# AugmentariumLab/VolumeRenderer

Measured on AMD Instinct MI355X. Metric: Mvoxels/s kd-tree compress+decode, higher is better.
Workload: dtype u8; 1 GPU; 2048x2048x1920 uint8 volume per GPU as 960 bricks of 256x256x128, rm_volume, tolerance 1, maxEpochs 2, VolumeKdtree build + levelCut

## Files before the change

### include/vrhip.h

```cpp
#ifndef VRHIP_H
#define VRHIP_H

#include <stdint.h>

#ifdef __cplusplus
extern "C" {
#endif

typedef int32_t vr_status;
enum {
    VR_OK = 0,
    VR_ERR_INVALID = -1,
    VR_ERR_NO_DEVICE = -2,
    VR_ERR_OOM = -3,
    VR_ERR_IO = -4,
    VR_ERR_STATE = -5,
    VR_ERR_FORMAT = -6,
    VR_ERR_UNSUPPORTED = -7
};

enum {
    VR_VARIANT_RECOVER = 0,
    VR_VARIANT_GUARDED = 1,
    VR_VARIANT_MIDRANGE = 2
// ... 267 lines not shown
vr_status vr_stream_create(void **stream);
vr_status vr_stream_destroy(void *stream);
vr_status vr_stream_synchronize(void *stream);
vr_status vr_stream_wait_event(void *stream, void *event);
vr_status vr_event_create(void **event);
vr_status vr_event_destroy(void *event);
vr_status vr_event_record(void *event, void *stream);
vr_status vr_event_synchronize(void *event);
vr_status vr_event_elapsed_ms(void *start_event, void *end_event, float *ms);
vr_status vr_malloc_host(void **host, int64_t bytes);
vr_status vr_free_host(void *host);
vr_status vr_upload_async(void *dst_dev, const void *src_host, int64_t bytes, void *stream);
vr_status vr_download_async(void *dst_host, const void *src_dev, int64_t bytes, void *stream);

vr_status vr_brickset_last_timings(vr_brickset *bs, float phases_ms[5]);

vr_status vr_brickset_set_concurrency(vr_brickset *bs, int32_t level_loop_streams);

vr_status vr_brickset_set_compaction(vr_brickset *bs, int32_t on_build);

vr_status vr_brickset_set_switch(vr_brickset *bs, const char *name, int32_t value);
vr_status vr_debug_set(const char *name, int32_t value);

#ifdef __cplusplus
}
#endif
#endif
```

### volumerenderer_amd/_lib.py

```python
import ctypes as C
import os

HERE = os.path.dirname(os.path.abspath(__file__))
LIB_PATH = os.path.join(HERE, "libvrhip.so")

VR_OK = 0
STATUS = {0: "VR_OK", -1: "VR_ERR_INVALID", -2: "VR_ERR_NO_DEVICE", -3: "VR_ERR_OOM", -4: "VR_ERR_IO",
          -5: "VR_ERR_STATE", -6: "VR_ERR_FORMAT", -7: "VR_ERR_UNSUPPORTED"}
VARIANT_RECOVER, VARIANT_GUARDED, VARIANT_MIDRANGE = 0, 1, 2
RENDER_COMPOSITE, RENDER_ISOSURFACE, RENDER_PARTIAL, RENDER_SHADED, RENDER_PROJECTION = 0, 1, 2, 3, 4
PROJECT_MAX, PROJECT_MIN, PROJECT_MEAN = 0, 1, 2
SLICE_NEAREST, SLICE_LINEAR = 0, 1


class VrError(RuntimeError):
    def __init__(self, status, what=""):
        self.status = status
        super().__init__("%s: %s (%d)" % (what, STATUS.get(status, "?"), status))


class TreeInfo(C.Structure):
    _fields_ = [("X", C.c_int64), ("Y", C.c_int64), ("Z", C.c_int64),
                ("orig_tree_depth", C.c_int32), ("max_tree_depth", C.c_int32),
                ("num_active_nodes", C.c_int64), ("tree_bytes", C.c_int64),
                ("tolerance", C.c_int32), ("max_epochs", C.c_int32), ("variant", C.c_int32),
                ("num_reverts", C.c_int32), ("max_error_before", C.c_int32), ("max_error_after", C.c_int32),
                ("mean_l1_after", C.c_double), ("zero_run_rewrites", C.c_int32), ("est_exact_segments", C.c_int32)]


class Camera(C.Structure):
    _fields_ = [("pos", C.c_float * 3), ("front", C.c_float * 3), ("up", C.c_float * 3),
                ("fov_deg", C.c_float), ("z_near", C.c_float), ("z_far", C.c_float)]


class RenderParams(C.Structure):
# ... 118 lines not shown
    "vr_compositor_create_from_comm": (_I32, [C.POINTER(_P), _P, _I32, _I32, _I32, _I32]),
    "vr_compositor_create_with_transport": (_I32, [C.POINTER(_P), _P, _P, _I32, _I32, _I32, _I32]),
    "vr_compositor_composite": (_I32, [_P, _P, _I32, C.POINTER(Camera), C.POINTER(RenderParams), _P, _P]),
    "vr_compositor_composite_tf": (_I32, [_P, _P, _I32, C.POINTER(Camera), C.POINTER(RenderParams),
                                          C.POINTER(TransferFunctionDesc), _P, _P]),
    "vr_compositor_composite_proj": (_I32, [_P, _P, C.POINTER(Projection), _P, _P]),
    "vr_compositor_destroy": (_I32, [_P]),
    "vr_stream_create": (_I32, [C.POINTER(_P)]),
    "vr_stream_destroy": (_I32, [_P]),
    "vr_stream_synchronize": (_I32, [_P]),
    "vr_stream_wait_event": (_I32, [_P, _P]),
    "vr_event_create": (_I32, [C.POINTER(_P)]),
    "vr_event_destroy": (_I32, [_P]),
    "vr_event_record": (_I32, [_P, _P]),
    "vr_event_synchronize": (_I32, [_P]),
    "vr_event_elapsed_ms": (_I32, [_P, _P, C.POINTER(C.c_float)]),
    "vr_malloc_host": (_I32, [C.POINTER(_P), _I64]),
    "vr_free_host": (_I32, [_P]),
    "vr_upload_async": (_I32, [_P, _P, _I64, _P]),
    "vr_download_async": (_I32, [_P, _P, _I64, _P]),
    "vr_brickset_last_timings": (_I32, [_P, C.POINTER(C.c_float)]),
    "vr_brickset_set_concurrency": (_I32, [_P, C.c_int32]),
    "vr_brickset_set_switch": (_I32, [_P, C.c_char_p, C.c_int32]),
    "vr_brickset_set_compaction": (_I32, [_P, C.c_int32]),
    "vr_debug_set": (_I32, [C.c_char_p, C.c_int32]),
}

_lib = None


def lib():
    global _lib
    if _lib is None:
        if not os.path.exists(LIB_PATH):
            raise ImportError("libvrhip.so is missing: run `python -c 'import __graft_entry__ as g; g.build()'` "
                              "(hipcc --offload-arch=gfx950).  There is no CPU fallback.")
        import torch
        L = C.CDLL(LIB_PATH)
        for name, (res, args) in SIGNATURES.items():
            fn = getattr(L, name)
            fn.restype = res
            fn.argtypes = args
        _lib = L
    return _lib


# ... 4 lines not shown
```

### volumerenderer_amd/codec.py

```python
import ctypes as C
import os

import numpy as np
import torch

from . import _lib
from ._lib import VrError, check


def _stream_ptr(stream=None):
    s = stream if stream is not None else torch.cuda.current_stream()
    return C.c_void_p(s.cuda_stream)


def _as_dev_u8(x):
    if isinstance(x, np.ndarray):
        x = torch.from_numpy(np.ascontiguousarray(x, dtype=np.uint8))
    if not isinstance(x, torch.Tensor) or x.dtype != torch.uint8:
        raise TypeError("expected a uint8 numpy array or torch tensor")
    if not x.is_cuda:
        x = x.cuda()
    return x.contiguous()


# ... 11 lines not shown
        self.dims = tuple(int(v) for v in dims)
        self.voxels_per_brick = self.dims[0] * self.dims[1] * self.dims[2]
        self._keep = None

    def __del__(self):
        try:
            if self._h:
                self._L.vr_brickset_destroy(self._h)
                self._h = None
        except Exception:
            pass

    def set_error_tolerance(self, tol):
        check(self._L.vr_brickset_set_error_tolerance(self._h, int(tol)), "setErrorTolerance")

    def set_max_epochs(self, e):
        check(self._L.vr_brickset_set_max_epochs(self._h, int(e)), "setMaxEpochs")

    def set_compaction(self, on_build=True):
        check(self._L.vr_brickset_set_compaction(self._h, 1 if on_build else 0), "vr_brickset_set_compaction")

    def set_switch(self, name, value=1):
        check(self._L.vr_brickset_set_switch(self._h, name.encode(), int(value)), "vr_brickset_set_switch(%s)" % name)

    def build(self, voxels, stream=None):
        v = _as_dev_u8(voxels)
        if v.numel() != self.num_bricks * self.voxels_per_brick:
            raise ValueError("voxel buffer has %d bytes, expected %d" % (v.numel(), self.num_bricks * self.voxels_per_brick))
        self._keep = v
        check(self._L.vr_brickset_build(self._h, C.c_void_p(v.data_ptr()), _stream_ptr(stream)), "vr_brickset_build")
        return self

    def info(self, brick=0):
        ti = _lib.TreeInfo()
        check(self._L.vr_brickset_info(self._h, int(brick), C.byref(ti)), "vr_brickset_info")
        return {k: getattr(ti, k) for k, _ in ti._fields_}

    def tree(self, brick=0):
        n = self.info(brick)["tree_bytes"]
        out = np.empty(n, np.uint8)
        check(self._L.vr_brickset_get_tree(self._h, int(brick), out.ctypes.data, n), "vr_brickset_get_tree")
        return out

    def distance_map(self, brick=0):
        n = self.info(brick)["max_tree_depth"] + 1
        out = np.empty(n, np.uint8)
# ... 254 lines not shown
```

### volumerenderer_amd/csrc/brickset.h

```cpp
#pragma once
#include "kd_common.h"
#include "../../include/vrhip.h"
#include <algorithm>
#include <string>
#include <vector>

namespace vr {

struct Stream2 {
    uint8_t *temp = nullptr;
    uint8_t *codes = nullptr;
    uint8_t *recon[3] = {nullptr, nullptr, nullptr};
    Ctrl *ctrl = nullptr;
    uint8_t *tree = nullptr;
    uint8_t *treeCompact = nullptr;
};

#define EST_R0_BUDGET 8
struct Switches {
    bool decodeWalk = false;
    bool decodeFineV1 = false;
    bool decodeQuad = false;
    bool noSkipBlocks = false;
    bool noUniformBlocks = false;
    bool estExactBounds = false;
    int estBudget = EST_R0_BUDGET;
    bool noUniformDecode = false;
};

#define VR_LOD_SLOTS 4
struct LodSlot {
    int32_t *dev = nullptr;
    int32_t *host = nullptr;
    uint8_t *idxValCut = nullptr;
    uint32_t *decTables = nullptr;
    uint8_t *rankVals = nullptr;
    int64_t *obDev = nullptr;
    int64_t *obHost = nullptr;
    vr_pool_entry *tabHost = nullptr;
    int64_t tabCap = 0;
    hipEvent_t done = nullptr;
    bool pending = false;
};

struct BrickSet {
    int32_t B = 0;
    Switches sw;
    Geom g{};
    TilePlan tile{};
// ... 110 lines not shown
```

### volumerenderer_amd/csrc/capi.hip

```cpp
#include "../../include/vrhip.h"
#include "brickset.h"
#include "raymarch.h"
#include <math.h>
#include <stdio.h>
#include <stdlib.h>
#include <string.h>
#include <algorithm>
#include <array>
#include <atomic>
#include <map>
#include <mutex>
#include <new>

using namespace vr;

struct vr_brickset { BrickSet s; };

#define HIPCHK(x) do { hipError_t e_ = (x); if (e_ != hipSuccess) return e_ == hipErrorOutOfMemory ? VR_ERR_OOM : VR_ERR_NO_DEVICE; } while (0)

static bool device_ok()
{
    int n = 0;
    hipError_t e = hipGetDeviceCount(&n);
    if ((e != hipSuccess || n <= 0) && getenv("VRHIP_DEBUG"))
// ... 80 lines not shown
    hipFree(s.treeCompact);
    hipFree(s.temp); hipFree(s.codes);
    for (int i = 0; i < 3; ++i) hipFree(s.recon[i]);
    hipFree(s.ctrl); hipFree(s.tree);
    s = Stream2();
}

static vr_status alloc_stream2(BrickSet &b, Stream2 &s)
{
    const size_t B = (size_t)b.B;
    HIPCHK(hipMalloc(&s.ctrl, B * sizeof(Ctrl)));
    HIPCHK(hipMemset(s.ctrl, 0, B * sizeof(Ctrl)));
    HIPCHK(hipMalloc(&s.tree, B * (size_t)b.treeCap));
    return VR_OK;
}

static void free_encoder_buffers(BrickSet &b)
{
    auto drop = [](auto *&p) { if (p) hipFree(p); p = nullptr; };
    Stream2 *ss[2] = {&b.mid, &b.rng};
    for (Stream2 *s : ss) {
        drop(s->temp); drop(s->codes);
        for (int i = 0; i < 3; ++i) drop(s->recon[i]);
    }
    for (int i = 0; i < 2; ++i) { drop(b.mmMin[i]); drop(b.mmMax[i]); }
    drop(b.blockErr); drop(b.estSumm); drop(b.blockErrR); drop(b.estSummR); drop(b.blockL1); drop(b.blockFlag); drop(b.blockFlagR); drop(b.blockAlive); drop(b.blockVal); drop(b.blockSpine); drop(b.blockSpineR);
    drop(b.chainLut); drop(b.blockTot); drop(b.blockOff); drop(b.blockOff64); drop(b.idxBase);
    b.encoderReady = false;
}

static vr_status alloc_encoder_buffers(BrickSet &b)
{
    const size_t B = (size_t)b.B;
    b.leafless = leafless_build(b);
    b.reconStride = b.leafless ? b.leafStride / 2 : b.leafStride;
    b.codeStride = b.leafless ? b.leafStride / 4 + 16 : ((b.heapStride + 15) / 16) * 4;
    HIPCHK(hipMalloc(&b.mid.temp, B * (size_t)b.heapStride));
    HIPCHK(hipMalloc(&b.mid.codes, B * (size_t)b.codeStride));
    for (int i = 0; i < 3; ++i) HIPCHK(hipMalloc(&b.mid.recon[i], B * (size_t)b.reconStride));
    if (b.variant == VR_VARIANT_MIDRANGE) {
        if (!b.rng.ctrl) HIPCHK(hipMalloc(&b.rng.ctrl, B * sizeof(Ctrl)));
        if (!b.rng.tree) HIPCHK(hipMalloc(&b.rng.tree, B * (size_t)b.treeCap));
        HIPCHK(hipMalloc(&b.rng.temp, B * (size_t)b.heapStride));
        HIPCHK(hipMalloc(&b.rng.codes, B * (size_t)b.codeStride));
        for (int i = 0; i < 3; ++i) HIPCHK(hipMalloc(&b.rng.recon[i], B * (size_t)b.reconStride));
    }
// ... 64 lines not shown
{
    if (!out || !dims || num_bricks <= 0) return VR_ERR_INVALID;
    if (tolerance < 0 || max_epochs < 0 || variant < 0 || variant > 2) return VR_ERR_INVALID;
    for (int k = 0; k < 3; ++k) if (dims[k] <= 0) return VR_ERR_INVALID;
    if (max_epochs > VR_MAX_EPOCHS) return VR_ERR_UNSUPPORTED;
    bool general = !pow2(dims[0]) || !pow2(dims[1]) || !pow2(dims[2]) || dims[0] > 1024 || dims[1] > 1024 || dims[2] > 1024;
    if (dims[0] > (1ll << 20) || dims[1] > (1ll << 20) || dims[2] > (1ll << 20) || dims[0] * dims[1] * dims[2] >= (1ll << 32))
        return VR_ERR_UNSUPPORTED;
    if (!device_ok()) return VR_ERR_NO_DEVICE;
    vr_brickset *h = new (std::nothrow) vr_brickset();
    if (!h) return VR_ERR_OOM;
    BrickSet &b = h->s;
    b.B = num_bricks;
    {
        Switches &w = b.sw;
        w.decodeWalk = getenv("VRHIP_DECODE_WALK") != nullptr;
        w.decodeFineV1 = getenv("VRHIP_DECODE_FINE_V1") != nullptr;
        w.decodeQuad = getenv("VRHIP_DECODE_QUAD") != nullptr;
        w.noSkipBlocks = getenv("VRHIP_NO_SKIP_BLOCKS") != nullptr;
        w.noUniformBlocks = getenv("VRHIP_NO_UNIFORM_BLOCKS") != nullptr;
        w.noUniformDecode = getenv("VRHIP_NO_UNIFORM_DECODE") != nullptr;
        w.estExactBounds = getenv("VRHIP_EST_EXACT_BOUNDS") != nullptr;
        if (const char *eb = getenv("VRHIP_EST_BUDGET")) { const int v = atoi(eb); if (v >= 0) w.estBudget = v; }
    }
    make_geom(b.g, dims);
    b.D = b.g.D;
    if (b.D > 31) { delete h; return VR_ERR_UNSUPPORTED; }
    b.idx64 = b.D > 28 || (getenv("VRHIP_FORCE_IDX64") && b.D >= 12);
    if (b.idx64) general = true;
    if (b.idx64 && num_bricks != 1 && b.D > 28) { delete h; return VR_ERR_UNSUPPORTED; }
    b.generalGeom = general;
    b.maxDepth = b.D + VR_CHAIN_LEVELS;
    b.tolerance = tolerance; b.maxEpochs = max_epochs; b.variant = variant;
    b.K = b.D < 6 ? b.D : 6;
    b.Ds = b.D - b.K;
    b.heapStride = (int64_t)1 << (b.D + 1);
    b.leafStride = (int64_t)1 << b.D;
    b.codeStride = ((b.heapStride + 15) / 16) * 4;
    b.reconStride = b.leafStride;
    const int64_t numMax = b.heapStride - 1 + VR_CHAIN_LEVELS * b.leafStride;
    b.treeCap = ((numMax + 15) / 16 + 2) * 4 + 256;
    if (b.D >= 12) {
        const int64_t gappedBytes = ((int64_t)1 << (b.D - 12)) * 2320 * 4 + 256;
        if (gappedBytes > b.treeCap) b.treeCap = gappedBytes;
    }
    b.nIdx = (int64_t)1 << b.Ds;
// ... 16 lines not shown
        if (e == hipSuccess && !general) e = upload(b.spread, make_spread(b.g));
        for (int i = 0; i < 8 && e == hipSuccess; ++i) e = hipEventCreate(&b.ev[i]);
        if (e != hipSuccess) rc = e == hipErrorOutOfMemory ? VR_ERR_OOM : VR_ERR_NO_DEVICE;
    }
    if (rc != VR_OK) { vr_brickset_destroy(h); return rc; }
    b.hostCtrl.resize(b.B);
    b.openTreeBytes.assign(b.B, -1);
    *out = h;
    return VR_OK;
}

vr_status vr_brickset_set_switch(vr_brickset *h, const char *name, int32_t value)
{
    if (!h || !name) return VR_ERR_INVALID;
    Switches &w = h->s.sw;
    const bool on = value != 0;
    if (!strcmp(name, "decode_walk")) w.decodeWalk = on;
    else if (!strcmp(name, "decode_fine_v1")) w.decodeFineV1 = on;
    else if (!strcmp(name, "decode_quad")) w.decodeQuad = on;
    else if (!strcmp(name, "no_skip_blocks")) w.noSkipBlocks = on;
    else if (!strcmp(name, "no_uniform_blocks")) w.noUniformBlocks = on;
    else if (!strcmp(name, "no_uniform_decode")) w.noUniformDecode = on;
    else if (!strcmp(name, "est_exact_bounds")) w.estExactBounds = on;
    else return VR_ERR_INVALID;
    return VR_OK;
}

vr_status vr_brickset_set_compaction(vr_brickset *h, int32_t on_build)
{
    if (!h) return VR_ERR_INVALID;
    h->s.compactOnBuild = on_build != 0;
    return VR_OK;
}

vr_status vr_debug_set(const char *name, int32_t value)
{
    if (!name) return VR_ERR_INVALID;
    if (!strcmp(name, "skip_grid_v1")) { vr::g_skipGridV1.store(value ? 1 : 0); return VR_OK; }
    if (!strcmp(name, "reslice_tile_w")) {
        if (value != 8 && value != 16 && value != 64) return VR_ERR_INVALID;
        vr::g_resliceTileLog2.store(value == 8 ? 3 : (value == 16 ? 4 : 6));
        return VR_OK;
    }
    if (!strcmp(name, "hist_plain")) { vr::g_histPlain.store(value ? 1 : 0); return VR_OK; }
    return VR_ERR_INVALID;
}

// ... 1018 lines not shown
```

### volumerenderer_amd/csrc/kd_encode.hip

```cpp
#include "brickset.h"
#include <math.h>
#include <stdio.h>
#include <stdlib.h>
#include <string.h>

namespace vr {

#define FILL_NODES_PER_BLOCK 1024
#define EMIT_RANKS_PER_BLOCK 256

template <bool FROM_VOXELS>
__global__ void __launch_bounds__(256)
k_pyramid(Geom g, int dLeaf, int L, const uint8_t *__restrict__ vox, const uint8_t *__restrict__ inMin,
          const uint8_t *__restrict__ inMax, int64_t inStride, uint8_t *__restrict__ temp, int64_t heapStride,
          uint8_t *__restrict__ tempRange, uint8_t *__restrict__ outMin, uint8_t *__restrict__ outMax,
          int64_t outStride, const uint32_t *__restrict__ srcIdx)
{
    __shared__ uint8_t smn[2][1024], smx[2][1024];
    const int brick = blockIdx.y;
    const uint32_t n = 1u << L;
    const uint32_t base = blockIdx.x << L;
    uint8_t *T = temp + (int64_t)brick * heapStride;
    uint8_t *TR = tempRange ? tempRange + (int64_t)brick * heapStride : nullptr;
    for (uint32_t i = threadIdx.x; i < n; i += blockDim.x) {
// ... 259 lines not shown
    if (threadIdx.x) return;
    c.constBrick = 0; c.constVal = 0; c.zeroRun = 0;
    if (rootMin) {
        const int mn = rootMin[(int64_t)blockIdx.x * mmStride], mx = rootMax[(int64_t)blockIdx.x * mmStride];
        c.constBrick = mn == mx ? 1 : 0;
        c.constVal = mn;
    }
    c.currentDistance = c.currentError = c.currentDF = c.currentStepSize = 0.0;
    c.previousDistance = c.previousError = c.previousDF = c.previousStepSize = 0.0;
    c.errMinus = c.errPlus = 0;
    c.statL1 = 0;
    c.numActive = 0;
    c.epoch = 0; c.active = 0; c.fillThisEpoch = 0;
    c.cur = 0; c.prev = 1; c.pendingEqual = 0;
    c.par = 0; c.ra = 1; c.rb = 2;
    c.altValid = 0; c.altSel = 0; c.altDist = 0;
    c.numReverts = 0; c.maxErrBefore = 0; c.maxErrAfter = 0;
    c.estS = 0; c.estC = 0; c.estTbase = 0; c.estFallbacks = 0; c.estSeg = 0; c.estDone = 0; c.emitOverflow = 0;
    for (int i = 0; i < VR_MAX_DEPTH + 8; ++i) c.distanceMap[i] = 0;
}

#define EST_SEG 1024
#define EST_CAND 8
#define EST_ROUNDS 5
#define EST_HEAD 4096

#define est_at(ci, seg) (((int64_t)(ci) * summStride + (int64_t)(seg)) * 4)

__device__ __forceinline__ uint32_t wave_incl_scan_u32(uint32_t v, int lane)
{
    (void)lane;
    return wave_incl_scan_add_dpp(v);
}

__device__ __forceinline__ uint32_t lane_u32(uint32_t v, int l) { return (uint32_t)__builtin_amdgcn_readlane((int)v, l); }
__device__ __forceinline__ unsigned long long lane_u64(unsigned long long v, int l)
{
    return (unsigned long long)lane_u32((uint32_t)v, l) | ((unsigned long long)lane_u32((uint32_t)(v >> 32), l) << 32);
}

#define EST_STAGE_NODES 4096
__device__ inline void est_exact_chain(const uint8_t *__restrict__ T, const uint8_t *__restrict__ P, int d, uint32_t lo,
                                       uint32_t hi, unsigned long long &S, uint32_t &C, int lane, const SkipBlocks &sk, int brick,
                                       uint8_t *stage = nullptr)
{
    const uint32_t len = hi - lo;
    const bool staged = stage && d > 0 && len >= 64u && len <= (uint32_t)EST_STAGE_NODES && (len & 63u) == 0u && (lo & 31u) == 0u;
// ... 88 lines not shown
            c.estDone = 0;
            c.estTbase = est_window_base((long long)(S / (2ull * C + 1ull)), 4);
        }
    }
}

__device__ __forceinline__ uint32_t seg_incl_scan_add_dpp(uint32_t v)
{
    v = row_incl_scan_add_dpp(v);
    return v + dpp_u32<0x142, 0xa>(0, v);
}
__device__ __forceinline__ int seg_max_i32_dpp(int v)
{
    v = row_max_i32_dpp(v);
    return max(v, (int)dpp_u32<0x142, 0xa>(0x80000000u, (uint32_t)v));
}
__device__ __forceinline__ int seg_min_i32_dpp(int v)
{
    v = row_min_i32_dpp(v);
    return min(v, (int)dpp_u32<0x142, 0xa>(0x7FFFFFFFu, (uint32_t)v));
}

template <bool QUADS>
__global__ void __launch_bounds__(256)
k_est_summ(int d, int nc, Ctrl *ctrls, const uint8_t *__restrict__ temp, int64_t heapStride, ReconBufs rb,
           int64_t leafStride, uint32_t *__restrict__ summ, int64_t summStride, SkipBlocks sk)
{
    constexpr int L = 32, SPW = 64 / L, NP = EST_SEG / 2 / L, TW = NP / 2, PW = NP / 4;
    const int brick = blockIdx.y, lane = threadIdx.x & 63, row = lane / L, rl = lane % L;
    const Ctrl &c = ctrls[brick];
    const uint32_t n = 1u << d;
    const int cConst = c.constBrick, cDone = c.estDone, cSeg = c.estSeg, cPar = c.par, cTbase = c.estTbase;
    if (cConst || cDone) return;
    const uint8_t *Tl = temp + (int64_t)brick * heapStride + ((int64_t)1 << d) + rl * (4 * TW);
    const uint8_t *Pl = (cPar == 0 ? rb.b[0] : (cPar == 1 ? rb.b[1] : rb.b[2])) + (int64_t)brick * leafStride + rl * (4 * PW);
    const uint32_t nseg = n / EST_SEG, step = gridDim.x * (4u * SPW);
    const uint32_t g0 = (uint32_t)cSeg + (blockIdx.x * 4u + (threadIdx.x >> 6)) * SPW;
    uint4 tN[TW / 4], pN[PW / 4];
    auto fetch = [&](uint32_t g) {
        const uint32_t s = g + (uint32_t)row;
        const bool live = s < nseg && !skip_block(sk, brick, d, s * EST_SEG);
#pragma unroll
        for (int j = 0; j < TW / 4; ++j) tN[j] = make_uint4(0, 0, 0, 0);
#pragma unroll
        for (int j = 0; j < PW / 4; ++j) pN[j] = make_uint4(0, 0, 0, 0);
        if (live) {
#pragma unroll
            for (int j = 0; j < TW / 4; ++j) tN[j] = ld16(Tl + (size_t)s * EST_SEG + 16 * j);
#pragma unroll
            for (int j = 0; j < PW / 4; ++j) pN[j] = ld16(Pl + (size_t)s * (EST_SEG / 2) + 16 * j);
        }
    };
    fetch(g0);
    const int Tbase = cTbase;
    uint32_t *out = summ + (int64_t)brick * summStride * (4 * EST_CAND);
    for (uint32_t g = g0; g < nseg; g += step) {
    uint32_t tw[TW], pw[PW];
#pragma unroll
    for (int j = 0; j < TW / 4; ++j) { tw[4 * j] = tN[j].x; tw[4 * j + 1] = tN[j].y; tw[4 * j + 2] = tN[j].z; tw[4 * j + 3] = tN[j].w; }
#pragma unroll
// ... 113 lines not shown
                amax = __builtin_elementwise_max(amax, low);
                bmin = __builtin_elementwise_min(bmin, pk_mad(cc, two2, low));
            }
        }
        const int low1 = low.x, low2 = low.y, cc1 = cc.x, cc2 = cc.y;
        lowT = low1 + low2; ccT = cc1 + cc2;
        a = max((int)amax.x, max((int)amax.y, 0) + low1);
        b = min((int)bmin.x, min((int)bmin.y, 0) + low1 + 2 * cc1);
        }
        const uint32_t sT = (uint32_t)(2 * Th * ccT - lowT);
        const uint32_t packed = sT | ((uint32_t)ccT << 20);
        const uint32_t incl = seg_incl_scan_add_dpp(packed), excl = incl - packed;
        const int s0 = (int)(excl & 0xFFFFFu), c0 = (int)(excl >> 20);
        a += 2 * Th * c0 - s0;
        b += 2 * (Th + 1) * c0 - s0;
        a = seg_max_i32_dpp(a);
        b = seg_min_i32_dpp(b);
        if (segLive && rl == L - 1)
            *(uint4 *)(out + est_at(ci, seg)) = make_uint4(incl & 0xFFFFFu, incl >> 20, (uint32_t)a, (uint32_t)b);
    }
    }
}

__global__ void __launch_bounds__(64)
k_est_walk(int d, int maxEpochs, int nc, int ncNext, int lastRound, int budget, Ctrl *ctrls, const uint8_t *__restrict__ temp, int64_t heapStride, ReconBufs rb,
           int64_t leafStride, const uint32_t *__restrict__ summ, int64_t summStride, SkipBlocks sk)
{
    const int brick = blockIdx.x, lane = threadIdx.x;
    Ctrl &c = ctrls[brick];
    const uint8_t *T = temp + (int64_t)brick * heapStride + ((int64_t)1 << d);
    const uint8_t *P = rb.b[c.par] + (int64_t)brick * leafStride;
    const uint32_t n = 1u << d, nseg = n / EST_SEG;
    const uint32_t *sm = summ + (int64_t)brick * summStride * (4 * EST_CAND);
    if (c.constBrick || c.estDone) return;
    __shared__ __attribute__((aligned(16))) uint8_t stage[EST_STAGE_NODES + EST_STAGE_NODES / 2];
    unsigned long long S = c.estS;
    uint32_t C = c.estC;
    const int Tbase = c.estTbase;
    long long Tc = (long long)(S / (2ull * C + 1ull));
    uint32_t seg = (uint32_t)c.estSeg;
    int fallbacks = 0;
    uint32_t preSeg = 0xFFFFFFFFu;
    long long preCi = -1;
    uint4 pre[4];
#pragma unroll
    for (int j = 0; j < 4; ++j) pre[j] = make_uint4(0, 0, 0x80000000u, 0x7FFFFFFFu);
    const auto fetch = [&](long long ci_, uint32_t seg_, uint4 (&r)[4]) {
        const uint32_t k0 = seg_ + 4u * (uint32_t)lane;
#pragma unroll
        for (int j = 0; j < 4; ++j) {
            r[j] = make_uint4(0, 0, 0x80000000u, 0x7FFFFFFFu);
            if (k0 + (uint32_t)j < nseg) r[j] = *(const uint4 *)(sm + est_at((int)ci_, k0 + (uint32_t)j));
        }
    };
    while (seg < nseg) {
        const long long ci = Tc - Tbase;
        if (ci < 0 || ci >= nc || (budget >= 0 && !lastRound && fallbacks > budget)) {
            if (!lastRound) {
                if (lane == 0) {
                    c.estS = S; c.estC = C; c.estSeg = (int)seg;
                    c.estTbase = est_window_base(Tc, ncNext);
                    c.estFallbacks += fallbacks;
                }
                return;
            }
            est_exact_chain(T, P, d, seg * EST_SEG, n, S, C, lane, sk, brick);
            fallbacks += (int)(nseg - seg);
            break;
        }
        uint4 r[4];
        if (preSeg == seg && preCi == ci) {
#pragma unroll
            for (int j = 0; j < 4; ++j) r[j] = pre[j];
        } else fetch(ci, seg, r);
        preSeg = seg + 256u; preCi = ci;
        fetch(ci, preSeg, pre);
        const uint32_t k0 = seg + 4u * (uint32_t)lane;
        const uint32_t ssL = r[0].x + r[1].x + r[2].x + r[3].x, scL = r[0].y + r[1].y + r[2].y + r[3].y;
        const uint32_t si = wave_incl_scan_u32(ssL, lane), sci = wave_incl_scan_u32(scL, lane);
        uint32_t eS = si - ssL, eC = sci - scL;
        int failJ = 4;
        uint32_t fS = 0, fC = 0;
#pragma unroll
        for (int j = 0; j < 4; ++j) {
            const long long S0 = (long long)S + (long long)eS;
// ... 1789 lines not shown
    }
    const int64_t s = (int64_t)blockIdx.x * 256 + threadIdx.x;
    if (s < nIdx) {
        idxOff[(int64_t)brick * nIdx + s] = VR_IDX_DEAD;
        idxVal[(int64_t)brick * nIdx + s] = (uint8_t)v;
    }
}

__global__ void k_const_finish_range(int D, Ctrl *ctrlsR, uint8_t *treeR, int64_t treeCap, const unsigned long long *brickOff = nullptr,
                                     int64_t compactCap = 0)
{
    Ctrl &c = ctrlsR[blockIdx.x];
    if (threadIdx.x || !c.constBrick) return;
    if (brickOff && brickOff[gridDim.x] > (unsigned long long)compactCap) return;
    const int v = c.constVal;
    for (int d = 0; d <= D; ++d) c.distanceMap[d] = 0;
    c.numActive = v ? 3 : 1;
    *(uint32_t *)(treeR + (brickOff ? (int64_t)brickOff[blockIdx.x] : (int64_t)blockIdx.x * treeCap)) = v ? 0x3Cu : 0x03u;
    c.numReverts = 0; c.maxErrBefore = 0; c.maxErrAfter = 0; c.statL1 = 0; c.emitOverflow = 0;
}

static inline unsigned cdiv(int64_t a, int64_t b) { return (unsigned)((a + b - 1) / b); }

static void compress_stream(BrickSet *bs, Stream2 &s0, hipStream_t st, const uint8_t *rootMin, const uint8_t *rootMax,
                            int64_t mmStride, SkipBlocks sk, unsigned long long *blockErr, void *estSumm0,
                            int b0 = 0, int nb = -1)
{
    const int D = bs->D, B = nb < 0 ? bs->B : nb;
    struct { Ctrl *ctrl; uint8_t *temp, *codes; uint8_t *recon[3]; } s;
    s.ctrl = s0.ctrl + b0; s.temp = s0.temp + (int64_t)b0 * bs->heapStride; s.codes = s0.codes + (int64_t)b0 * bs->codeStride;
    for (int i = 0; i < 3; ++i) s.recon[i] = s0.recon[i] + (int64_t)b0 * bs->reconStride;
    blockErr += (int64_t)b0 * bs->nErrBlk;
    const int64_t errPlane = (int64_t)bs->B * bs->nErrBlk;
    void *estSumm = (uint32_t *)estSumm0 + (int64_t)b0 * bs->estSummStride * (4 * EST_CAND);
    if (sk.flag) sk.flag += (int64_t)b0 * sk.nBlk;
    if (rootMin) { rootMin += (int64_t)b0 * mmStride; rootMax += (int64_t)b0 * mmStride; }
    ReconBufs rb{{s.recon[0], s.recon[1], s.recon[2]}};
    const int guarded = bs->variant != 0;
    hipLaunchKernelGGL(k_ctrl_init, dim3(B), dim3(64), 0, st, s.ctrl, rootMin, rootMax, mmStride);
    if (bs->maxEpochs <= 0) {
        for (int i = 0; i < 3; ++i) hipMemsetAsync(s.recon[i], 0, (size_t)B * bs->reconStride, st);
        hipMemsetAsync(s.codes, 0, (size_t)B * bs->codeStride, st);
    }
    for (int d = 0; d <= D; ++d) {
        const int64_t n = (int64_t)1 << d;
        if (sk.flag && d == D - 1)
            hipLaunchKernelGGL(k_fill_const_leaves, dim3(cdiv(sk.nBlk, 256), B), dim3(256), 0, st, D, s.ctrl, s.temp,
                               bs->heapStride, sk);
        hipLaunchKernelGGL(k_est_head, dim3(B), dim3(64), 0, st, d, bs->maxEpochs, s.ctrl, s.temp, bs->heapStride, rb,
                           bs->reconStride, sk);
        if (n > EST_HEAD) {
            const int64_t nseg = n / EST_SEG - EST_HEAD / EST_SEG;
            for (int r = 0; r < EST_ROUNDS; ++r) {
                const int nc = r < 2 ? 4 : EST_CAND, ncNext = r + 1 < 2 ? 4 : EST_CAND;
                const unsigned gx = r == 0 ? cdiv(nseg, 32) : (cdiv(nseg, 8) < 64 ? cdiv(nseg, 8) : 64);
                const bool quads = r == 0 && !bs->sw.estExactBounds;
                hipLaunchKernelGGL(quads ? k_est_summ<true> : k_est_summ<false>, dim3(gx, B), dim3(256), 0, st, d, nc, s.ctrl, s.temp,
                                   bs->heapStride, rb, bs->reconStride, (uint32_t *)estSumm, bs->estSummStride, sk);
                hipLaunchKernelGGL(k_est_walk, dim3(B), dim3(64), 0, st, d, bs->maxEpochs, nc, ncNext,
                                   r == EST_ROUNDS - 1 ? 1 : 0, quads ? bs->sw.estBudget : -1, s.ctrl, s.temp, bs->heapStride, rb, bs->reconStride,
                                   (const uint32_t *)estSumm, bs->estSummStride, sk);
            }
        }
        for (int e = 0; e < bs->maxEpochs; ++e) {
            if (n >= 4096)
            {
                const int iters = n / 4096 >= 512 ? FILL_ITERS : (n / 4096 >= 64 ? (FILL_ITERS < 4 ? FILL_ITERS : 4) : 1);
                hipLaunchKernelGGL((bs->leafless && d == D) ? k_fill16<false> : k_fill16<true>, dim3(cdiv(n / 4096, iters), B), dim3(256), 0, st,
                                   d, bs->maxEpochs, s.ctrl, s.temp, s.codes, bs->heapStride, bs->codeStride, rb, bs->reconStride, blockErr,
                                   bs->nErrBlk, sk, errPlane, iters);
            }
            else
                hipLaunchKernelGGL(k_fill, dim3(cdiv(n, FILL_NODES_PER_BLOCK), B), dim3(256), 0, st, d, s.ctrl, s.temp,
                                   s.codes, bs->heapStride, bs->codeStride, rb, bs->reconStride, blockErr, bs->nErrBlk);
            hipLaunchKernelGGL(k_control, dim3(B), dim3(64), 0, st, d, bs->maxEpochs, guarded, s.ctrl, s.temp,
                               bs->heapStride, rb, bs->reconStride, blockErr, bs->nErrBlk, errPlane, (bs->leafless && d == D) ? 1 : 0);
        }
        hipLaunchKernelGGL(k_level_end, dim3(B), dim3(64), 0, st, d, s.ctrl);
    }
}

__global__ void k_fix_chain_distances(int D, int maxDepth, Ctrl *ctrls, Ctrl *ctrlsR)
{
    if (threadIdx.x) return;
// ... 114 lines not shown
            uint8_t *oMin = bs->mmMin[round & 1], *oMax = bs->mmMax[round & 1];
            if (round == 0)
                hipLaunchKernelGGL(k_pyramid<true>, dim3((unsigned)nblk, B), dim3(256), 0, st, bs->g, dLeaf, L, vox,
                                   inMin, inMax, inStride, bs->mid.temp, bs->heapStride, mr ? bs->rng.temp : nullptr,
                                   oMin, oMax, oStride, bs->generalGeom ? bs->srcIdx : nullptr);
            else
                hipLaunchKernelGGL(k_pyramid<false>, dim3((unsigned)nblk, B), dim3(256), 0, st, bs->g, dLeaf, L, vox,
                                   inMin, inMax, inStride, bs->mid.temp, bs->heapStride, mr ? bs->rng.temp : nullptr,
                                   oMin, oMax, oStride, nullptr);
            dLeaf -= L;
            rootMinP = oMin; rootMaxP = oMax;
            if (dLeaf == 0) break;
            inMin = oMin; inMax = oMax; inStride = oStride;
            ++round;
        }
    }
    hipEventRecord(bs->ev[1], st);
    dbg_sync(st, "pyramid");
    const bool constOk = bs->maxEpochs >= 1 && bs->tolerance >= 1 && D >= 1;
    const uint8_t *cMin = constOk ? rootMinP : nullptr, *cMax = constOk ? rootMaxP : nullptr;
    const SkipBlocks sk{skipOn ? bs->blockFlag : nullptr, (int64_t)1 << (D >= 12 ? D - 12 : 0), D - 2};
    const SkipBlocks skR{skipOn && mr ? bs->blockFlagR : nullptr, sk.nBlk, D - 2};
    const bool forkR = mr && bs->blockErrR && bs->estSummR && ensure_aux(bs, 1) == 1;
    if (forkR) {
        hipEventRecord(bs->evFork, st);
        hipStreamWaitEvent(bs->aux, bs->evFork, 0);
        compress_stream(bs, bs->rng, bs->aux, cMin, cMax, rootStride, skR, bs->blockErrR, bs->estSummR);
        hipEventRecord(bs->evJoin, bs->aux);
    }
    int parts = bs->levelLoopStreams;
    if (parts > 4) parts = 4;
    if (mr || B < 16 * parts || parts < 2) parts = 1;
    if (parts > 1) parts = 1 + ensure_aux(bs, parts - 1);
    if (parts > 1) {
        hipEventRecord(bs->evFork, st);
        for (int p = 1; p < parts; ++p) {
            const int b0 = (int)((int64_t)B * p / parts), b1 = (int)((int64_t)B * (p + 1) / parts);
            hipStreamWaitEvent(bs->auxN[p - 1], bs->evFork, 0);
            compress_stream(bs, bs->mid, bs->auxN[p - 1], cMin, cMax, rootStride, sk, bs->blockErr, bs->estSumm, b0, b1 - b0);
            hipEventRecord(bs->evJoinN[p - 1], bs->auxN[p - 1]);
        }
        compress_stream(bs, bs->mid, st, cMin, cMax, rootStride, sk, bs->blockErr, bs->estSumm, 0, (int)((int64_t)B / parts));
        for (int p = 1; p < parts; ++p) hipStreamWaitEvent(st, bs->evJoinN[p - 1], 0);
    } else
    compress_stream(bs, bs->mid, st, cMin, cMax, rootStride, sk, bs->blockErr, bs->estSumm);
    if (forkR) hipStreamWaitEvent(st, bs->evJoin, 0);
    else if (mr) compress_stream(bs, bs->rng, st, cMin, cMax, rootStride, skR, bs->blockErr, bs->estSumm);
    hipEventRecord(bs->ev[2], st);
    dbg_sync(st, "compress");
    hipLaunchKernelGGL(k_chain_lut, dim3(1), dim3(256), 0, st, kernel_tolerance(*bs), bs->maxDepth - D, bs->chainLut);
    ReconBufs rb{{bs->mid.recon[0], bs->mid.recon[1], bs->mid.recon[2]}};
    ReconBufs rbR{{bs->rng.recon[0], bs->rng.recon[1], bs->rng.recon[2]}};
    int pruneFrom = D - 1;
    bs->fineHas.assign((size_t)B, 0);
    fine_has_changed(*bs);
    if (fused) {
        PruneEmitArgs pa;
        pa.sk = sk; pa.skR = skR;
        pa.D = D; pa.tol = kernel_tolerance(*bs); pa.maxDepth = bs->maxDepth; pa.ctrls = bs->mid.ctrl;
        pa.temp = bs->mid.temp; pa.codes = bs->mid.codes;
        pa.heapStride = bs->heapStride; pa.codeStride = bs->codeStride; pa.leafStride = bs->reconStride;
        pa.rb = rb; pa.subTok = bs->blockOff; pa.nEmitBlk = bs->nEmitBlk; pa.blockL1 = bs->blockL1;
// ... 65 lines not shown
```

Measured before the change: 289,100 Mvoxels/s.

## Compact still-active bricks into work lists for estimator rounds

The estimator walk kernel now appends each brick that needs another refinement round to a device-side work list with an atomic counter. In later rounds the non-quad estimator summary kernel reads that list and runs a fixed grid of rows that loop over only the listed bricks, instead of launching one row per brick and having finished bricks exit early. This is meant to cut launch and idle-block cost as bricks converge. In exchange it adds a memset per stream, atomics, and an indirect loop, plus a debug API for reading the list counts.

```diff
diff --git a/include/vrhip.h b/include/vrhip.h
--- a/include/vrhip.h
+++ b/include/vrhip.h
@@ -313,6 +313,9 @@
 vr_status vr_brickset_set_switch(vr_brickset *bs, const char *name, int32_t value);
 vr_status vr_debug_set(const char *name, int32_t value);
 
+#define VR_EST_ROUNDS 5
+vr_status vr_brickset_work_list_counts(vr_brickset *bs, int32_t range_stream, uint32_t *est, int64_t est_len);
+
 #ifdef __cplusplus
 }
 #endif
diff --git a/volumerenderer_amd/_lib.py b/volumerenderer_amd/_lib.py
--- a/volumerenderer_amd/_lib.py
+++ b/volumerenderer_amd/_lib.py
@@ -11,6 +11,7 @@
 RENDER_COMPOSITE, RENDER_ISOSURFACE, RENDER_PARTIAL, RENDER_SHADED, RENDER_PROJECTION = 0, 1, 2, 3, 4
 PROJECT_MAX, PROJECT_MIN, PROJECT_MEAN = 0, 1, 2
 SLICE_NEAREST, SLICE_LINEAR = 0, 1
+EST_ROUNDS = 5
 
 
 class VrError(RuntimeError):
@@ -175,6 +176,7 @@
     "vr_brickset_last_timings": (_I32, [_P, C.POINTER(C.c_float)]),
     "vr_brickset_set_concurrency": (_I32, [_P, C.c_int32]),
     "vr_brickset_set_switch": (_I32, [_P, C.c_char_p, C.c_int32]),
+    "vr_brickset_work_list_counts": (_I32, [_P, C.c_int32, _P, C.c_int64]),
     "vr_brickset_set_compaction": (_I32, [_P, C.c_int32]),
     "vr_debug_set": (_I32, [C.c_char_p, C.c_int32]),
 }
diff --git a/volumerenderer_amd/codec.py b/volumerenderer_amd/codec.py
--- a/volumerenderer_amd/codec.py
+++ b/volumerenderer_amd/codec.py
@@ -57,6 +57,13 @@
 
     def set_switch(self, name, value=1):
         check(self._L.vr_brickset_set_switch(self._h, name.encode(), int(value)), "vr_brickset_set_switch(%s)" % name)
+
+    def work_list_counts(self, range_stream=False):
+        levels = self.info(0)["orig_tree_depth"] + 1
+        est = np.zeros((levels, _lib.EST_ROUNDS), np.uint32)
+        check(self._L.vr_brickset_work_list_counts(self._h, 1 if range_stream else 0, est.ctypes.data_as(C.c_void_p), est.size),
+              "vr_brickset_work_list_counts")
+        return est
 
     def build(self, voxels, stream=None):
         v = _as_dev_u8(voxels)
diff --git a/volumerenderer_amd/csrc/brickset.h b/volumerenderer_amd/csrc/brickset.h
--- a/volumerenderer_amd/csrc/brickset.h
+++ b/volumerenderer_amd/csrc/brickset.h
@@ -14,7 +14,11 @@
     Ctrl *ctrl = nullptr;
     uint8_t *tree = nullptr;
     uint8_t *treeCompact = nullptr;
+    uint32_t *wlList = nullptr;
+    uint32_t *wlCnt = nullptr;
+    int32_t wlRanges = 0;
 };
+#define VR_WL_RANGES 4
 
 #define EST_R0_BUDGET 8
 struct Switches {
@@ -25,6 +29,8 @@
     bool noUniformBlocks = false;
     bool estExactBounds = false;
     int estBudget = EST_R0_BUDGET;
+    int noWorkLists = 0;
+    int workListWgs = 0;
     bool noUniformDecode = false;
 };
 
diff --git a/volumerenderer_amd/csrc/capi.hip b/volumerenderer_amd/csrc/capi.hip
--- a/volumerenderer_amd/csrc/capi.hip
+++ b/volumerenderer_amd/csrc/capi.hip
@@ -126,6 +126,8 @@
     for (Stream2 *s : ss) {
         drop(s->temp); drop(s->codes);
         for (int i = 0; i < 3; ++i) drop(s->recon[i]);
+        drop(s->wlList); drop(s->wlCnt);
+        s->wlRanges = 0;
     }
     for (int i = 0; i < 2; ++i) { drop(b.mmMin[i]); drop(b.mmMax[i]); }
     drop(b.blockErr); drop(b.estSumm); drop(b.blockErrR); drop(b.estSummR); drop(b.blockL1); drop(b.blockFlag); drop(b.blockFlagR); drop(b.blockAlive); drop(b.blockVal); drop(b.blockSpine); drop(b.blockSpineR);
@@ -236,6 +238,8 @@
         w.noUniformDecode = getenv("VRHIP_NO_UNIFORM_DECODE") != nullptr;
         w.estExactBounds = getenv("VRHIP_EST_EXACT_BOUNDS") != nullptr;
         if (const char *eb = getenv("VRHIP_EST_BUDGET")) { const int v = atoi(eb); if (v >= 0) w.estBudget = v; }
+        if (const char *nl = getenv("VRHIP_NO_WORK_LISTS")) w.noWorkLists = atoi(nl) & 1;
+        if (const char *wg = getenv("VRHIP_WORK_LIST_WGS")) { const int v = atoi(wg); if (v >= 0 && v <= 65535) w.workListWgs = v; }
     }
     make_geom(b.g, dims);
     b.D = b.g.D;
@@ -298,7 +302,28 @@
     else if (!strcmp(name, "no_uniform_blocks")) w.noUniformBlocks = on;
     else if (!strcmp(name, "no_uniform_decode")) w.noUniformDecode = on;
     else if (!strcmp(name, "est_exact_bounds")) w.estExactBounds = on;
+    else if (!strcmp(name, "no_work_lists")) { if (value < 0 || value > 1) return VR_ERR_INVALID; w.noWorkLists = value; }
+    else if (!strcmp(name, "work_list_wgs")) { if (value < 0 || value > 65535) return VR_ERR_INVALID; w.workListWgs = value; }
     else return VR_ERR_INVALID;
+    return VR_OK;
+}
+
+vr_status vr_brickset_work_list_counts(vr_brickset *h, int32_t range_stream, uint32_t *est, int64_t est_len)
+{
+    if (!h || !est || range_stream < 0 || range_stream > 1) return VR_ERR_INVALID;
+    BrickSet &b = h->s;
+    if (!b.built || b.foreign) return VR_ERR_STATE;
+    const Stream2 &s = range_stream ? b.rng : b.mid;
+    const int64_t nEst = (int64_t)(b.D + 1) * VR_EST_ROUNDS;
+    if (est_len < nEst) return VR_ERR_INVALID;
+    std::fill(est, est + est_len, 0u);
+    HIPCHK(hipStreamSynchronize((hipStream_t)b.lastStream));
+    if (s.wlRanges > 0 && s.wlCnt) {
+        std::vector<uint32_t> host((size_t)(nEst * s.wlRanges));
+        HIPCHK(hipMemcpy(host.data(), s.wlCnt, host.size() * sizeof(uint32_t), hipMemcpyDeviceToHost));
+        for (int r = 0; r < s.wlRanges; ++r)
+            for (int64_t i = 0; i < nEst; ++i) est[i] += host[(size_t)(nEst * r + i)];
+    }
     return VR_OK;
 }
 
diff --git a/volumerenderer_amd/csrc/kd_encode.hip b/volumerenderer_amd/csrc/kd_encode.hip
--- a/volumerenderer_amd/csrc/kd_encode.hip
+++ b/volumerenderer_amd/csrc/kd_encode.hip
@@ -305,7 +305,7 @@
 
 #define EST_SEG 1024
 #define EST_CAND 8
-#define EST_ROUNDS 5
+#define EST_ROUNDS VR_EST_ROUNDS
 #define EST_HEAD 4096
 
 #define est_at(ci, seg) (((int64_t)(ci) * summStride + (int64_t)(seg)) * 4)
@@ -440,12 +440,12 @@
 }
 
 template <bool QUADS>
-__global__ void __launch_bounds__(256)
-k_est_summ(int d, int nc, Ctrl *ctrls, const uint8_t *__restrict__ temp, int64_t heapStride, ReconBufs rb,
-           int64_t leafStride, uint32_t *__restrict__ summ, int64_t summStride, SkipBlocks sk)
+__device__ __forceinline__ void
+est_summ_brick(const int brick, const uint32_t tid, int d, int nc, Ctrl *ctrls, const uint8_t *__restrict__ temp, int64_t heapStride, const ReconBufs &rb,
+               int64_t leafStride, uint32_t *__restrict__ summ, int64_t summStride, const SkipBlocks &sk)
 {
     constexpr int L = 32, SPW = 64 / L, NP = EST_SEG / 2 / L, TW = NP / 2, PW = NP / 4;
-    const int brick = blockIdx.y, lane = threadIdx.x & 63, row = lane / L, rl = lane % L;
+    const int lane = tid & 63, row = lane / L, rl = lane % L;
     const Ctrl &c = ctrls[brick];
     const uint32_t n = 1u << d;
     const int cConst = c.constBrick, cDone = c.estDone, cSeg = c.estSeg, cPar = c.par, cTbase = c.estTbase;
@@ -453,7 +453,7 @@
     const uint8_t *Tl = temp + (int64_t)brick * heapStride + ((int64_t)1 << d) + rl * (4 * TW);
     const uint8_t *Pl = (cPar == 0 ? rb.b[0] : (cPar == 1 ? rb.b[1] : rb.b[2])) + (int64_t)brick * leafStride + rl * (4 * PW);
     const uint32_t nseg = n / EST_SEG, step = gridDim.x * (4u * SPW);
-    const uint32_t g0 = (uint32_t)cSeg + (blockIdx.x * 4u + (threadIdx.x >> 6)) * SPW;
+    const uint32_t g0 = (uint32_t)cSeg + (blockIdx.x * 4u + (tid >> 6)) * SPW;
     uint4 tN[TW / 4], pN[PW / 4];
     auto fetch = [&](uint32_t g) {
         const uint32_t s = g + (uint32_t)row;
@@ -613,9 +613,28 @@
     }
 }
 
+template <bool QUADS>
+__global__ void __launch_bounds__(256)
+k_est_summ(int d, int nc, Ctrl *ctrls, const uint8_t *__restrict__ temp, int64_t heapStride, ReconBufs rb,
+           int64_t leafStride, uint32_t *__restrict__ summ, int64_t summStride, SkipBlocks sk,
+           const uint32_t *__restrict__ list, const uint32_t *__restrict__ listCount)
+{
+    if (QUADS) {
+        est_summ_brick<QUADS>((int)blockIdx.y, threadIdx.x, d, nc, ctrls, temp, heapStride, rb, leafStride, summ, summStride, sk);
+        return;
+    }
+    const uint32_t count = list ? *listCount : gridDim.y;
+    uint32_t tid = threadIdx.x;
+    for (uint32_t i = blockIdx.y; i < count; i += gridDim.y) {
+        asm volatile("" : "+v"(tid));
+        est_summ_brick<QUADS>(__builtin_amdgcn_readfirstlane((int)(list ? list[i] : i)), tid, d, nc, ctrls, temp, heapStride, rb, leafStride, summ, summStride, sk);
+    }
+}
+
 __global__ void __launch_bounds__(64)
 k_est_walk(int d, int maxEpochs, int nc, int ncNext, int lastRound, int budget, Ctrl *ctrls, const uint8_t *__restrict__ temp, int64_t heapStride, ReconBufs rb,
-           int64_t leafStride, const uint32_t *__restrict__ summ, int64_t summStride, SkipBlocks sk)
+           int64_t leafStride, const uint32_t *__restrict__ summ, int64_t summStride, SkipBlocks sk,
+           uint32_t *__restrict__ nextList, uint32_t *__restrict__ nextCount)
 {
     const int brick = blockIdx.x, lane = threadIdx.x;
     Ctrl &c = ctrls[brick];
@@ -652,6 +671,7 @@
                     c.estS = S; c.estC = C; c.estSeg = (int)seg;
                     c.estTbase = est_window_base(Tc, ncNext);
                     c.estFallbacks += fallbacks;
+                    if (nextList) nextList[atomicAdd(nextCount, 1u)] = (uint32_t)brick;
                 }
                 return;
             }
@@ -2487,11 +2507,29 @@
 
 static inline unsigned cdiv(int64_t a, int64_t b) { return (unsigned)((a + b - 1) / b); }
 
+#define WL_ROWS 64
+
+static int ensure_work_lists(BrickSet *bs, Stream2 &s, int ranges)
+{
+    s.wlRanges = 0;
+    if (bs->sw.noWorkLists & 1) return 0;
+    if (!s.wlList && hipMalloc(&s.wlList, (size_t)2 * bs->B * sizeof(uint32_t)) != hipSuccess) return -3;
+    if (!s.wlCnt && hipMalloc(&s.wlCnt, (size_t)VR_WL_RANGES * (bs->D + 1) * EST_ROUNDS * sizeof(uint32_t)) != hipSuccess) return -3;
+    s.wlRanges = ranges;
+    return 0;
+}
+
 static void compress_stream(BrickSet *bs, Stream2 &s0, hipStream_t st, const uint8_t *rootMin, const uint8_t *rootMax,
                             int64_t mmStride, SkipBlocks sk, unsigned long long *blockErr, void *estSumm0,
-                            int b0 = 0, int nb = -1)
+                            int b0 = 0, int nb = -1, int range = 0)
 {
     const int D = bs->D, B = nb < 0 ? bs->B : nb;
+    const bool estLists = s0.wlRanges > range && s0.wlList && s0.wlCnt;
+    const int64_t wlSlice = (int64_t)(D + 1) * EST_ROUNDS;
+    uint32_t *const wlEstCnt = estLists ? s0.wlCnt + (int64_t)range * wlSlice : nullptr;
+    uint32_t *const wlEstList[2] = {estLists ? s0.wlList + b0 : nullptr, estLists ? s0.wlList + (int64_t)bs->B + b0 : nullptr};
+    const unsigned wlRows = bs->sw.workListWgs > 0 ? (unsigned)bs->sw.workListWgs : (unsigned)WL_ROWS;
+    if (estLists) hipMemsetAsync(wlEstCnt, 0, (size_t)wlSlice * sizeof(uint32_t), st);
     struct { Ctrl *ctrl; uint8_t *temp, *codes; uint8_t *recon[3]; } s;
     s.ctrl = s0.ctrl + b0; s.temp = s0.temp + (int64_t)b0 * bs->heapStride; s.codes = s0.codes + (int64_t)b0 * bs->codeStride;
     for (int i = 0; i < 3; ++i) s.recon[i] = s0.recon[i] + (int64_t)b0 * bs->reconStride;
@@ -2520,11 +2558,14 @@
                 const int nc = r < 2 ? 4 : EST_CAND, ncNext = r + 1 < 2 ? 4 : EST_CAND;
                 const unsigned gx = r == 0 ? cdiv(nseg, 32) : (cdiv(nseg, 8) < 64 ? cdiv(nseg, 8) : 64);
                 const bool quads = r == 0 && !bs->sw.estExactBounds;
-                hipLaunchKernelGGL(quads ? k_est_summ<true> : k_est_summ<false>, dim3(gx, B), dim3(256), 0, st, d, nc, s.ctrl, s.temp,
-                                   bs->heapStride, rb, bs->reconStride, (uint32_t *)estSumm, bs->estSummStride, sk);
+                const bool listed = estLists && r >= 1, lister = estLists && r + 1 < EST_ROUNDS;
+                hipLaunchKernelGGL(quads ? k_est_summ<true> : k_est_summ<false>, dim3(gx, listed ? wlRows : (unsigned)B), dim3(256), 0, st, d, nc, s.ctrl, s.temp,
+                                   bs->heapStride, rb, bs->reconStride, (uint32_t *)estSumm, bs->estSummStride, sk,
+                                   listed ? wlEstList[r & 1] : nullptr, listed ? wlEstCnt + d * EST_ROUNDS + r : nullptr);
                 hipLaunchKernelGGL(k_est_walk, dim3(B), dim3(64), 0, st, d, bs->maxEpochs, nc, ncNext,
                                    r == EST_ROUNDS - 1 ? 1 : 0, quads ? bs->sw.estBudget : -1, s.ctrl, s.temp, bs->heapStride, rb, bs->reconStride,
-                                   (const uint32_t *)estSumm, bs->estSummStride, sk);
+                                   (const uint32_t *)estSumm, bs->estSummStride, sk,
+                                   lister ? wlEstList[(r + 1) & 1] : nullptr, lister ? wlEstCnt + d * EST_ROUNDS + r + 1 : nullptr);
             }
         }
         for (int e = 0; e < bs->maxEpochs; ++e) {
@@ -2685,6 +2726,8 @@
     const SkipBlocks sk{skipOn ? bs->blockFlag : nullptr, (int64_t)1 << (D >= 12 ? D - 12 : 0), D - 2};
     const SkipBlocks skR{skipOn && mr ? bs->blockFlagR : nullptr, sk.nBlk, D - 2};
     const bool forkR = mr && bs->blockErrR && bs->estSummR && ensure_aux(bs, 1) == 1;
+    bs->mid.wlRanges = bs->rng.wlRanges = 0;
+    if (mr && ensure_work_lists(bs, bs->rng, 1) != 0) return -3;
     if (forkR) {
         hipEventRecord(bs->evFork, st);
         hipStreamWaitEvent(bs->aux, bs->evFork, 0);
@@ -2695,12 +2738,13 @@
     if (parts > 4) parts = 4;
     if (mr || B < 16 * parts || parts < 2) parts = 1;
     if (parts > 1) parts = 1 + ensure_aux(bs, parts - 1);
+    if (ensure_work_lists(bs, bs->mid, parts) != 0) return -3;
     if (parts > 1) {
         hipEventRecord(bs->evFork, st);
         for (int p = 1; p < parts; ++p) {
             const int b0 = (int)((int64_t)B * p / parts), b1 = (int)((int64_t)B * (p + 1) / parts);
             hipStreamWaitEvent(bs->auxN[p - 1], bs->evFork, 0);
-            compress_stream(bs, bs->mid, bs->auxN[p - 1], cMin, cMax, rootStride, sk, bs->blockErr, bs->estSumm, b0, b1 - b0);
+            compress_stream(bs, bs->mid, bs->auxN[p - 1], cMin, cMax, rootStride, sk, bs->blockErr, bs->estSumm, b0, b1 - b0, p);
             hipEventRecord(bs->evJoinN[p - 1], bs->auxN[p - 1]);
         }
         compress_stream(bs, bs->mid, st, cMin, cMax, rootStride, sk, bs->blockErr, bs->estSumm, 0, (int)((int64_t)B / parts));
```

Measured after the change: 291,900 Mvoxels/s (median of 6 runs). No clear change (+1.0%).
